# liruiw/GA-DDPG

Measured on AMD Instinct MI355X. Metric: DDPG grad-steps/sec (B=256, N=1024 pts), higher is better.
Workload: dtype f32 (3xbf16-split products, f32 accumulate)

## Files before the change

ga-ddpg_amd/csrc/gemm.hip:

```cpp
#include "common.hpp"
#include <mutex>
#include <type_traits>
#include <string.h>

typedef float f32x16 __attribute__((ext_vector_type(16)));

#ifndef GAD_STREAM_STORE_AUX
#define GAD_STREAM_STORE_AUX 0
#endif

#define KT 32

__device__ __forceinline__ float4 f4zero() { return make_float4(0.f, 0.f, 0.f, 0.f); }
__device__ __forceinline__ float4 f4sel(bool c, float4 a, float4 b) {
    return make_float4(c ? a.x : b.x, c ? a.y : b.y, c ? a.z : b.z, c ? a.w : b.w);
}
__device__ __forceinline__ float4 ldg4(const float* p) { return *reinterpret_cast<const float4*>(p); }

typedef unsigned gad_u32x4 __attribute__((ext_vector_type(4)));
__device__ __forceinline__ float4 buf_ld4(__amdgpu_buffer_rsrc_t r, int vo, int so) {
    const gad_u32x4 u = __builtin_amdgcn_raw_buffer_load_b128(r, vo, so, 0);
    return make_float4(__uint_as_float(u.x), __uint_as_float(u.y), __uint_as_float(u.z), __uint_as_float(u.w));
}
__device__ __forceinline__ float buf_ld(__amdgpu_buffer_rsrc_t r, int vo, int so) {
// ... 205 lines not shown
        if (d.gmode == 0) {
            g = d.G[(size_t)rr * d.g_pitch + ch];
        } else {
            const int grp = d.row_grp[rr];
            g = d.argmax[(size_t)grp * d.c + ch] == r ? d.dout[(size_t)grp * d.c + ch] : 0.f;
        }
        if (d.relu && !d.premasked) {
            const float y = d.scale ? fmaf(z, d.scale[ch], d.shift[ch]) : z;
            g = y > 0.f ? g : 0.f;
        }
        if (d.P) {
            const float w = d.row_w ? d.row_w[rr] : 1.f;
            g = d.P[ch] * g - w * fmaf(d.S[ch], z, d.Q[ch]);
        }
        v[j] = ok ? g : 0.f;
    }
    return make_float4(v[0], v[1], v[2], v[3]);
}

template <bool VEC>
__device__ __forceinline__ DzRaw dz_raw(const DzSrc& d, int r, bool valid, int off, int n, int nmax, int grp) {
    DzRaw o;
    o.z = f4zero(); o.a = make_int4(0, 0, 0, 0);
    if (!VEC) { o.g = dz_scalar4(d, r, valid, off, n, nmax); return o; }
    const int rr = valid ? r : 0;
    const int ch = off + (n < nmax ? n : 0);
    if (d.z) o.z = ldg4(d.z + (size_t)rr * d.z_pitch + ch);
    if (d.gmode == 0) {
        o.g = ldg4(d.G + (size_t)rr * d.g_pitch + ch);
    } else {
        o.a = *reinterpret_cast<const int4*>(d.argmax + (size_t)grp * d.c + ch);
        o.g = ldg4(d.dout + (size_t)grp * d.c + ch);
    }
    return o;
}

template <bool VEC, int VM = VMAX>
__device__ __forceinline__ float4 dz_finish(const DzSrc& d, const DzRaw& raw, int r, bool valid, int n, int nmax, float w,
                                            const float* vec) {
    if (!VEC) return raw.g;
    const bool inside = n < nmax;
    const int nn = inside ? n : 0;
    float4 g = raw.g;
    const float4 z = raw.z;
    if (d.gmode != 0) {
        g.x = raw.a.x == r ? g.x : 0.f; g.y = raw.a.y == r ? g.y : 0.f;
        g.z = raw.a.z == r ? g.z : 0.f; g.w = raw.a.w == r ? g.w : 0.f;
    }
    if (d.relu && !d.premasked) {
        float4 y = z;
        if (d.scale) {
            const float4 s = *reinterpret_cast<const float4*>(vec + nn), t = *reinterpret_cast<const float4*>(vec + VM + nn);
            y.x = fmaf(z.x, s.x, t.x); y.y = fmaf(z.y, s.y, t.y); y.z = fmaf(z.z, s.z, t.z); y.w = fmaf(z.w, s.w, t.w);
        }
        g.x = y.x > 0.f ? g.x : 0.f; g.y = y.y > 0.f ? g.y : 0.f;
        g.z = y.z > 0.f ? g.z : 0.f; g.w = y.w > 0.f ? g.w : 0.f;
    }
    if (d.coef) {
        const float4 P = *reinterpret_cast<const float4*>(vec + 2 * VM + nn);
        const float4 Q = *reinterpret_cast<const float4*>(vec + 3 * VM + nn);
        const float4 S = *reinterpret_cast<const float4*>(vec + 4 * VM + nn);
        g.x = P.x * g.x - w * fmaf(S.x, z.x, Q.x); g.y = P.y * g.y - w * fmaf(S.y, z.y, Q.y);
        g.z = P.z * g.z - w * fmaf(S.z, z.z, Q.z); g.w = P.w * g.w - w * fmaf(S.w, z.w, Q.w);
    }
    return f4sel(valid && inside, g, f4zero());
}

template <int VM = VMAX>
__device__ __forceinline__ void stage_dz_vecs(float* vec, const DzSrc& d, int off, int n) {
    if (!d.premasked) {
        stage_vec(vec, d.scale, off, n, 1.f);
        stage_vec(vec + VM, d.shift, off, n, 0.f);
    }
    for (int i = threadIdx.x; i < n; i += 256) {
        float P, Q, S;
        dz_coef(d, off + i, P, Q, S, first_workgroup());
        vec[2 * VM + i] = P; vec[3 * VM + i] = Q; vec[4 * VM + i] = S;
    }
}

static bool dz_vectorizable(const gad_dz_src& d, const int32_t* off, const int32_t* n_out, int ng) {
    bool ok = (d.z == nullptr || d.z_pitch % 4 == 0) && (d.gmode != 0 || d.g_pitch % 4 == 0) && (d.gmode == 0 || d.c % 4 == 0);
    for (int i = 0; i < ng; ++i) ok = ok && off[i] % 4 == 0 && n_out[i] % 4 == 0 && n_out[i] <= VMAX;
    return ok;
}

template <int DIM> struct PitchT { static constexpr int v = DIM + 1; };
template <int DIM> struct PitchD { static constexpr int v = DIM + 4; };

template <int DIM> __device__ __forceinline__ void unit_T(int u, int& i, int& kk) { i = u >> 3; kk = (u & 7) << 2; }
template <int DIM> __device__ __forceinline__ void unit_D(int u, int& kk, int& i) { kk = u / (DIM / 4); i = (u % (DIM / 4)) << 2; }

template <int DIM> __device__ __forceinline__ void store_T(float* t, int i, int kk, float4 v) {
    constexpr int P = PitchT<DIM>::v;
    t[(kk + 0) * P + i] = v.x; t[(kk + 1) * P + i] = v.y; t[(kk + 2) * P + i] = v.z; t[(kk + 3) * P + i] = v.w;
}
template <int DIM> __device__ __forceinline__ void store_D(float* t, int kk, int i, float4 v) {
    constexpr int P = PitchD<DIM>::v;
    *reinterpret_cast<float4*>(t + kk * P + i) = v;
}

template <int TM, int TN, int PA, int PB>
__device__ __forceinline__ void mfma_ktile(const float* __restrict__ As, const float* __restrict__ Bs, int am0,
                                           int bn0, int lane, f32x16 (&acc)[TM][TN]) {
    const int l31 = lane & 31, half = lane >> 5;
    constexpr int CH = 4, NCH = KT / 2 / CH;
    const float* ap = As + half * PA + am0 + l31;
    const float* bp = Bs + half * PB + bn0 + l31;
    float a[2][CH][TM], b[2][CH][TN];
    auto fetch = [&](int c, int buf) {
#pragma unroll
        for (int s = 0; s < CH; ++s) {
#pragma unroll
            for (int tm = 0; tm < TM; ++tm) a[buf][s][tm] = ap[(2 * (c * CH + s)) * PA + tm * 32];
#pragma unroll
            for (int tn = 0; tn < TN; ++tn) b[buf][s][tn] = bp[(2 * (c * CH + s)) * PB + tn * 32];
        }
    };
    fetch(0, 0);
#pragma unroll
    for (int c = 0; c < NCH; ++c) {
        if (c + 1 < NCH) fetch(c + 1, (c + 1) & 1);
        __builtin_amdgcn_sched_barrier(0);
#pragma unroll
        for (int s = 0; s < CH; ++s)
#pragma unroll
            for (int tm = 0; tm < TM; ++tm)
#pragma unroll
                for (int tn = 0; tn < TN; ++tn)
                    acc[tm][tn] = __builtin_amdgcn_mfma_f32_32x32x2f32(a[c & 1][s][tm], b[c & 1][s][tn], acc[tm][tn], 0, 0, 0);
    }
}

__device__ __forceinline__ int acc_row(int v, int half) { return (v & 3) + 8 * (v >> 2) + 4 * half; }

struct PoolEpi {
    unsigned long long* key;
    const int32_t* row_grp;
    const float* gamma;
    int C;
};

__device__ __forceinline__ unsigned pool_ord(float f) {
    const unsigned u = __float_as_uint(f);
    return u ^ ((unsigned)((int)u >> 31) | 0x80000000u);
}

__device__ __forceinline__ void pool_put(unsigned long long* keycol, int g, int C, float v, int row, bool partial) {
    const unsigned long long k = ((unsigned long long)pool_ord(v) << 32) | (unsigned long long)(0xffffffffu - (unsigned)row);
    if (partial) atomicMax(keycol + (size_t)g * C, k);
    else keycol[(size_t)g * C] = k;
}

struct PoolRun { int g; int part; float v; int row; };

template <int NC>
__device__ __forceinline__ void pool_rows(const float* zt, int pitch, int cstride, int i, int e, int row_base, const float (&sgn)[NC],
                                          float (&best)[NC], int (&brow)[NC]) {
    int r = i;
    for (; r + 2 <= e; r += 2) {
        float z0[NC], z1[NC];
#pragma unroll
        for (int c = 0; c < NC; ++c) { z0[c] = zt[r * pitch + c * cstride] * sgn[c]; z1[c] = zt[(r + 1) * pitch + c * cstride] * sgn[c]; }
#pragma unroll
        for (int c = 0; c < NC; ++c) {
            bool t = z0[c] > best[c]; best[c] = t ? z0[c] : best[c]; brow[c] = t ? row_base + r : brow[c];
            t = z1[c] > best[c]; best[c] = t ? z1[c] : best[c]; brow[c] = t ? row_base + r + 1 : brow[c];
        }
    }
    if (r < e) {
#pragma unroll
        for (int c = 0; c < NC; ++c) {
            const float z0 = zt[r * pitch + c * cstride] * sgn[c];
            const bool t = z0 > best[c]; best[c] = t ? z0 : best[c]; brow[c] = t ? row_base + r : brow[c];
        }
    }
}

__device__ __forceinline__ void pool_scan32(const float* zt, int pitch, int gl, int row_base, float sgn, PoolRun& c,
                                            unsigned long long* keycol, int C) {
    const int lane = threadIdx.x & 63;
    const int prev = __shfl_up(gl, 1, 64);
    const bool st = lane == 0 ? gl != c.g : gl != prev;
    const unsigned m = (unsigned)__ballot(st);
    int i = 0;
    while (i < 32) {
        if ((m >> i) & 1u) {
            if (c.g >= 0) pool_put(keycol, c.g, C, c.v, c.row, c.part != 0);
            c.g = __builtin_amdgcn_readlane(gl, i); c.part = 0; c.v = -INFINITY; c.row = row_base + i;
        }
        const unsigned rest = i < 31 ? m >> (i + 1) : 0u;
        const int e = rest ? i + 1 + __builtin_ctz(rest) : 32;
        if (c.g >= 0) {
            const float sg1[1] = {sgn};
            float bv[1] = {c.v};
            int br[1] = {c.row};
            pool_rows<1>(zt, pitch, 0, i, e, row_base, sg1, bv, br);
            c.v = bv[0]; c.row = br[0];
        }
        i = e;
    }
}

template <int NC>
__device__ __forceinline__ void pool_tile64(const float* zt, int pitch, int cstride, int gl, int row0, int n_live,
                                            const float (&sgn)[NC], int wave, int nw, int g_before, int g_after,
                                            unsigned long long* keycol, int C) {
    const int lane = threadIdx.x & 63;
    const int prev = __shfl_up(gl, 1, 64);
    const bool st = (lane == 0 || gl != prev) && lane < n_live;
    unsigned long long m = __ballot(st);
    int k = 0;
    while (m) {
        const int i = __builtin_ctzll(m);
        m &= m - 1;
        const int e = m ? __builtin_ctzll(m) : n_live;
        if ((k++ % nw) != wave) continue;
        const int g = __builtin_amdgcn_readlane(gl, i);
        float best[NC];
        int brow[NC];
#pragma unroll
        for (int c = 0; c < NC; ++c) { best[c] = -INFINITY; brow[c] = row0 + i; }
        pool_rows<NC>(zt, pitch, cstride, i, e, row0, sgn, best, brow);
        const bool partial = (i == 0 && g == g_before) || (e == n_live && g == g_after);
#pragma unroll
        for (int c = 0; c < NC; ++c) pool_put(keycol + c * cstride, g, C, best[c], brow[c], partial);
    }
}

struct Groups {
    int n; int aoff[GAD_MAX_GROUPS]; int woff[GAD_MAX_GROUPS]; int ooff[GAD_MAX_GROUPS]; int nout[GAD_MAX_GROUPS];
};

template <int WM, int WN, int TN, bool STORE = false>
__device__ __forceinline__ void block_column_atomics(float* red, const float (&c0)[TN], const float (&c1)[TN], int lane,
                                                     int wm, int wn, int col0, int col_limit, double* out0,
                                                     double* out1) {
    constexpr int BN = WN * TN * 32;
    __syncthreads();
#pragma unroll
    for (int tn = 0; tn < TN; ++tn) {
        const float s0 = c0[tn] + __shfl_xor(c0[tn], 32, 64);
        const float s1 = c1[tn] + __shfl_xor(c1[tn], 32, 64);
        if (lane < 32) {
            const int cl = wn * TN * 32 + tn * 32 + lane;
            red[wm * BN + cl] = s0;
            red[(WM + wm) * BN + cl] = s1;
        }
    }
    __syncthreads();
    const int tid = threadIdx.x;
    if (tid < BN && col0 + tid < col_limit) {
        float s0 = 0.f, s1 = 0.f;
#pragma unroll
        for (int w = 0; w < WM; ++w) { s0 += red[w * BN + tid]; s1 += red[(WM + w) * BN + tid]; }
        if (STORE) {
            out0[col0 + tid] = (double)s0;
            out1[col0 + tid] = (double)s1;
        } else {
            atomic_add_f64(out0 + col0 + tid, (double)s0);
            atomic_add_f64(out1 + col0 + tid, (double)s1);
        }
    }
}

template <int WM, int WN, int TM, int TN, int XM, bool POOL, bool DET = false>
__global__ __launch_bounds__(256) void gemm_fwd_kernel(XSrc x, Groups gr, const int32_t* __restrict__ n_rows_dev,
                                                        int n_rows_static, const float* __restrict__ row_w,
                                                        const float* __restrict__ W, int Kp,
                                                        float* __restrict__ zout, int zout_pitch,
                                                        double* __restrict__ stat_sum,
                                                        double* __restrict__ stat_sq, int stat_stride, PoolEpi pe,
                                                        unsigned long long* __restrict__ ts) {
    KTimer kt(ts);
    constexpr int BM = WM * TM * 32, BN = WN * TN * 32;
    constexpr int PA = PitchT<BM>::v, PB = PitchT<BN>::v;
    constexpr int UA = BM * 8 / 256, UB = BN * 8 / 256;
    constexpr int TILE = KT * PA + KT * PB;
    constexpr int SM = ((TILE + 3) & ~3) + 2 * BM + 2 * VMAX;
    static_assert(TILE >= 2 * WM * BN, "reduction scratch must fit in the tile LDS");
    __shared__ __attribute__((aligned(16))) float smem[SM];
    float* As = smem;
    float* Bs = smem + KT * PA;
    float* wS = smem + ((TILE + 3) & ~3);
    int32_t* ptS = reinterpret_cast<int32_t*>(wS + BM);
    float* sv = wS + 2 * BM;
    float* tv = sv + VMAX;

    const int tid = threadIdx.x, lane = tid & 63, wave = tid >> 6;
    const int wm = wave / WN, wn = wave % WN;
    const int g = blockIdx.z;
    const int zoff = gr.aoff[g], n_out = gr.nout[g], ooff = gr.ooff[g];
    const float* Wg = W + gr.woff[g];
    const int n0 = blockIdx.y * BN;
    if (n0 >= n_out) return;
    const int n_rows = n_rows_dev ? min(*n_rows_dev, n_rows_static) : n_rows_static;
    if ((int)(blockIdx.x * BM) >= n_rows) return;
    const int nk = (Kp + KT - 1) / KT;
    const int bulk = XM == 0 ? x.c_in : x.feat_c;

    float csum[TN], csq[TN];
#pragma unroll
    for (int t = 0; t < TN; ++t) { csum[t] = 0.f; csq[t] = 0.f; }

    int row0 = blockIdx.x * BM;
    XRaw ra[UA];
    float4 rb[UB];
    auto load_tile = [&](int kt) {
        const int k0 = kt * KT;
        const bool tail = k0 + KT > bulk;
#pragma unroll
        for (int it = 0; it < UA; ++it) {
            int i, kk; unit_T<BM>(it * 256 + tid, i, kk);
            const int r = row0 + i;
            const bool ok = r < n_rows && (k0 + kk < Kp);
            ra[it] = x_raw<XM>(x, r, ok, zoff, k0 + kk, tail, XM == 1 ? ptS[i] : 0);
        }
#pragma unroll
        for (int it = 0; it < UB; ++it) {
            int j, kk; unit_T<BN>(it * 256 + tid, j, kk);
            const int n = n0 + j;
            const bool ok = n < n_out && (k0 + kk < Kp);
            rb[it] = ldg4(Wg + (size_t)(ok ? n : 0) * Kp + (ok ? k0 + kk : 0));
        }
    };
    auto store_tile = [&](int kt) {
        const int k0 = kt * KT;
#pragma unroll
        for (int it = 0; it < UA; ++it) {
            int i, kk; unit_T<BM>(it * 256 + tid, i, kk);
            const int r = row0 + i;
            const bool ok = r < n_rows && (k0 + kk < Kp);
            store_T<BM>(As, i, kk, x_finish<XM>(x, ra[it], ok, k0 + kk, sv, tv));
        }
#pragma unroll
        for (int it = 0; it < UB; ++it) {
            int j, kk; unit_T<BN>(it * 256 + tid, j, kk);
            const bool ok = (n0 + j) < n_out && (k0 + kk < Kp);
            store_T<BN>(Bs, j, kk, f4sel(ok, rb[it], f4zero()));
        }
    };
    bool preloaded = false;
    if (XM == 0) { load_tile(0); preloaded = true; }
    if (XM == 0 && x.affine) stage_affine<256>(sv, tv, x, zoff, x.c_in);
    for (; row0 < n_rows; row0 += gridDim.x * BM) {
        f32x16 acc[TM][TN];
#pragma unroll
        for (int a = 0; a < TM; ++a)
#pragma unroll
            for (int b = 0; b < TN; ++b)
#pragma unroll
// ... 296 lines not shown
                    an = *reinterpret_cast<const float4*>(As + 8 * (j + 1));
                    bn0 = *reinterpret_cast<const float4*>(Bs + 8 * (j + 1));
                    bn1 = *reinterpret_cast<const float4*>(Bs + 32 * P + 8 * (j + 1));
                }
                acc[0] = __builtin_amdgcn_mfma_f32_32x32x2f32(a4.x, b0.x, acc[0], 0, 0, 0);
                acc[1] = __builtin_amdgcn_mfma_f32_32x32x2f32(a4.x, b1.x, acc[1], 0, 0, 0);
                acc[0] = __builtin_amdgcn_mfma_f32_32x32x2f32(a4.y, b0.y, acc[0], 0, 0, 0);
                acc[1] = __builtin_amdgcn_mfma_f32_32x32x2f32(a4.y, b1.y, acc[1], 0, 0, 0);
                acc[0] = __builtin_amdgcn_mfma_f32_32x32x2f32(a4.z, b0.z, acc[0], 0, 0, 0);
                acc[1] = __builtin_amdgcn_mfma_f32_32x32x2f32(a4.z, b1.z, acc[1], 0, 0, 0);
                acc[0] = __builtin_amdgcn_mfma_f32_32x32x2f32(a4.w, b0.w, acc[0], 0, 0, 0);
                acc[1] = __builtin_amdgcn_mfma_f32_32x32x2f32(a4.w, b1.w, acc[1], 0, 0, 0);
                a4 = an; b0 = bn0; b1 = bn1;
            }
            if (kt + 1 < nk) write_lds(kt + 1, nxtc);
            if (kt + 3 < nk) load_regs(kt + 3, nxtc);
            __syncthreads();
        };
        for (int kt = 0; kt < nk; kt += 2) {
            ktile(kt, S1);
            if (kt + 1 < nk) ktile(kt + 1, S0);
        }
        GAD_WPH(3);
        if (SP) {
#pragma unroll
            for (int t = 0; t < 2; ++t)
#pragma unroll
                for (int v = 0; v < 16; ++v) acc[t][v] = (v & 1) ? an[t][v] - acc[t][v] : acc[t][v] - an[t][v];
        }
        if (XM == 1) {
#pragma unroll
            for (int t = 0; t < 2; ++t) {
                const float* wx = W + (size_t)(n0 + wn * 64 + t * 32 + l31) * Kp + x.feat_c;
                const float w0 = wx[0], w1 = wx[1], w2 = wx[2];
#pragma unroll
                for (int v = 0; v < 16; ++v) {
                    const float4 q = *reinterpret_cast<const float4*>(dxS + 4 * (wm * 32 + acc_row(v, half)));
                    acc[t][v] = fmaf(q.x, w0, fmaf(q.y, w1, fmaf(q.z, w2, acc[t][v])));
                }
            }
        }
        if (POOL) {
            float* zt = smem;
#pragma unroll
            for (int t = 0; t < 2; ++t)
#pragma unroll
                for (int v = 0; v < 16; ++v) zt[(wm * 32 + acc_row(v, half)) * 129 + wn * 64 + t * 32 + l31] = acc[t][v];
            __syncthreads();
            const int gb = __builtin_amdgcn_readfirstlane(pg_before), ga = __builtin_amdgcn_readfirstlane(pg_after);
            pool_tile64<2>(zt + lane, 129, 64, pgl, row0, min(64, n_rows - row0), psgn, wave, 4, gb, ga, pe.key + n0 + lane, pe.C);
        }
        if (SP) {
#pragma unroll
        for (int t = 0; t < 2; ++t) {
            const int n = n0 + wn * 64 + t * 32 + l31;
            const int vzo = (4 * half * zout_pitch + n) * 4;
#pragma unroll
            for (int v = 0; v < 16; ++v)
                __builtin_amdgcn_raw_buffer_store_b32(__float_as_uint(acc[t][v]), zo_, vzo, (row0 + wm * 32 + (v & 3) + 8 * (v >> 2)) * zo_pitch4, 0);
        }
        __builtin_amdgcn_sched_barrier(0);
#pragma unroll
        for (int t = 0; t < 2; ++t) {
            float s1 = 0.f, s2 = 0.f;
#pragma unroll
            for (int v = 0; v < 16; ++v) {
                const float w = wS[wm * 32 + acc_row(v, half)];
                const float zv = acc[t][v];
                s1 = fmaf(w, zv, s1);
                s2 = fmaf(w * zv, zv, s2);
            }
            csum[t] += s1;
            csq[t] += s2;
        }
        } else {
#pragma unroll
        for (int t = 0; t < 2; ++t) {
            const int n = n0 + wn * 64 + t * 32 + l31;
            const int vzo = (4 * half * zout_pitch + n) * 4;
            float s1 = 0.f, s2 = 0.f;
#pragma unroll
            for (int v = 0; v < 16; ++v) {
                const int il = wm * 32 + acc_row(v, half);
                const float zv = acc[t][v];
                __builtin_amdgcn_raw_buffer_store_b32(__float_as_uint(zv), zo_, vzo, (row0 + wm * 32 + (v & 3) + 8 * (v >> 2)) * zo_pitch4, 0);
                const float w = wS[il];
                s1 = fmaf(w, zv, s1);
                s2 = fmaf(w * zv, zv, s2);
            }
            csum[t] += s1;
            csq[t] += s2;
        }
        }
        GAD_WPH(4);
    }
    if (stat_sum) {
        const int rep = blockIdx.x % GAD_STAT_REPLICAS;
        block_column_atomics<2, 2, 2>(smem, csum, csq, lane, wm, wn, n0, n_out, stat_sum + (size_t)rep * stat_stride,
                                      stat_sq + (size_t)rep * stat_stride);
    }
#ifdef GAD_W_PHASES
    __asm__ volatile("s_waitcnt vmcnt(0)" ::: "memory");
    GAD_WPH(5);
    GAD_WPH_STORE(ts);
    GAD_WKL_STORE(ts);
#endif
}

static int g_opt_fwd_wide = 1;
static int g_opt_dx_wide = 1, g_opt_dw_wide = 1;
static int g_opt_bwd_fused = 1;
static int g_opt_fwd_bn_prologue = 1;
static int g_opt_bwd_wide = 0;
static int g_opt_bwd_wide_slab = 4;
static int g_opt_dw_wide_wgs = 256;
static bool fits_i32_bytes(long long rows, int pitch_a, int pitch_b, int pitch_c, int pitch_d);
static bool fwd_wideable(const gad_gemm_fwd_args& a) {
    if (g_opt_deterministic || !g_opt_fwd_wide || a.n_groups != 1 || a.zin_off[0] != 0 || a.w_off[0] != 0 || a.out_off[0] != 0) return false;
    if (!fits_i32_bytes(a.n_rows, a.mode == 1 ? a.feat_c : a.zin_pitch, a.zout ? a.zout_pitch : 0, 0, 0)) return false;
    if (a.n_rows < 2048 || a.n_out[0] % 128 != 0 || a.ones_col >= 0) return false;
    if (a.mode == 2) return false;
    if (a.mode == 1)
        return g_opt_fwd_wide != 2 && !a.pool_key && a.act_c == 0 && a.feat_c % 32 == 0 && a.feat_c >= 32 && a.feat_c <= 512 &&
               a.Kp == ((a.feat_c + 3 + 7) & ~7);
    if (a.Kp % 32 != 0 || a.Kp > 512 || a.Kp != a.c_in) return false;
    return !a.extra && a.scale && a.shift && a.relu;
}
static bool fits_i32_bytes(long long rows, int pitch_a, int pitch_b, int pitch_c, int pitch_d) {
    int p = pitch_a > pitch_b ? pitch_a : pitch_b;
    p = p > pitch_c ? p : pitch_c;
    p = p > pitch_d ? p : pitch_d;
    return rows * (long long)p * 4 <= (1ll << 31);
}

template <int KJ, int TN, int XM, bool POOL, bool SP = false>
__global__ __launch_bounds__(512, 2) void gemm_fwd_stream_kernel(XSrc x, const int32_t* __restrict__ n_rows_dev,
                                                                  int n_rows_static, const float* __restrict__ row_w,
                                                                  const float* __restrict__ W, float* __restrict__ zout,
                                                                  double* __restrict__ stat_sum,
                                                                  double* __restrict__ stat_sq, int stat_stride, PoolEpi pe,
                                                                  unsigned long long* __restrict__ ts) {
#ifdef GAD_X_PHASES
    const long long kt_start = __builtin_readcyclecounter();
#else
    KTimer kt(ts);
#endif
    constexpr int KP = 8 * KJ, NO = 32 * TN, PW = KP + 4;
    constexpr bool RE = XM >= 2;
    constexpr int PK = RE ? XM - 1 : 0;
    constexpr bool ACT = XM == 0 || RE, GATHER = XM == 1 || RE;
    constexpr int NG = RE ? PK : KJ;
    static_assert(!RE || (KJ == 8 && !POOL), "recomputed input: 64 channels");
    static_assert(!SP || (XM == 0 && KJ == 8), "split-bf16: ACT input, 64 channels");
    constexpr int PB = 2 * KP + 16;
    __shared__ __attribute__((aligned(16))) float Ws[SP ? 3 * NO * PB / 4 : NO * PW];
    __shared__ __attribute__((aligned(16))) float sv[KP], tv[KP];
    __shared__ float red[2 * 8 * NO];
    __shared__ float pz[POOL ? 8 * 32 * 64 : 1];
    static_assert(!POOL || TN == 4, "pooled epilogue: 128 output columns");
    const int tid = threadIdx.x, lane = tid & 63;
    const int wave = __builtin_amdgcn_readfirstlane(tid >> 6);
    const int l31 = lane & 31, half = lane >> 5;
    const int n_rows = n_rows_dev ? min(*n_rows_dev, n_rows_static) : n_rows_static;
    const int n_slabs = (n_rows + 31) >> 5;
#if GAD_X_PHASES == 2
    long long st1, st2, st3, st4;
    __asm__ volatile("s_waitcnt lgkmcnt(0)" ::: "memory");
    GAD_PH_STAMP(st1);
#endif
    int stride = gridDim.x * 8;
    int slab = wave * gridDim.x + blockIdx.x;
    int slab_end = n_slabs;
    if (POOL) {
        const int nw = gridDim.x * 8, base = n_slabs / nw, rem = n_slabs - base * nw;
        slab_end = slab * base + min(slab, rem) + base + (slab < rem ? 1 : 0);
        slab = slab * base + min(slab, rem);
        stride = 1;
    }
    const bool store_z = zout != nullptr;
    const __amdgpu_buffer_rsrc_t zrsrc =
        __builtin_amdgcn_make_buffer_rsrc(store_z ? zout : const_cast<float*>(W), 0, store_z ? gad_nbytes(n_rows, NO * 4) : 0, 0x00020000);
    const int zlane = (4 * half * NO + l31) * 4;
    float psgn[2];
    PoolRun prun[2];
    const int range0 = slab * 32;
    int g_after = -1;
    if (POOL && slab < slab_end) {
        const int g0 = pe.row_grp[range0];
        const int part0 = range0 > 0 && pe.row_grp[range0 - 1] == g0;
        if (slab_end * 32 < n_rows) g_after = pe.row_grp[slab_end * 32];
#pragma unroll
        for (int p = 0; p < 2; ++p) {
            psgn[p] = pe.gamma[p * 64 + lane] < 0.f ? -1.f : 1.f;
            prun[p].g = g0; prun[p].part = part0; prun[p].v = -INFINITY; prun[p].row = range0;
        }
    }

    f32x2 csum[TN], csq[TN];
#pragma unroll
    for (int t = 0; t < TN; ++t) { csum[t] = f32x2{0.f, 0.f}; csq[t] = f32x2{0.f, 0.f}; }

    XRaw ra[NG], rn[NG];
    float4 w1f[RE ? 2 : 1][RE ? PK : 1];
    if (RE) {
#pragma unroll
        for (int b = 0; b < 2; ++b)
#pragma unroll
            for (int j = 0; j < PK; ++j) w1f[b][j] = ldg4(x.pre_W + (size_t)(32 * b + l31) * x.pre_Kp + 8 * j + 4 * half);
    }
    int pt_nxt = 0;
    auto load_pt = [&](int sl) {
        const int r = min(sl * 32 + l31, max(n_rows - 1, 0));
        return (GATHER && sl < n_slabs) ? x.row_pt[r] : 0;
    };
    auto load_slab = [&](int sl, int pt, XRaw (&dst)[NG]) {
        const int r = min(sl < n_slabs ? sl * 32 + l31 : 0, max(n_rows - 1, 0));
        if (GATHER) {
            struct F3 { float x, y, z; } __attribute__((packed, aligned(4)));
            const float4 f = ldg4(x.feat + (size_t)pt * 4);
            const F3 p = *reinterpret_cast<const F3*>(x.src_xyz + (size_t)pt * 3);
            const int grp = x.row_grp[r];
            float q0 = p.x, q1 = p.y, q2 = p.z;
            if (x.ctr_xyz) {
                const F3 c = *reinterpret_cast<const F3*>(x.ctr_xyz + (size_t)grp * 3);
                q0 = __fsub_rn(q0, c.x); q1 = __fsub_rn(q1, c.y); q2 = __fsub_rn(q2, c.z);
            }
            float a0 = 0.f, a1 = 0.f, a2 = 0.f, a3 = 0.f, a4 = 0.f, a5 = 0.f;
            if (x.action) {
                const float* ap = x.action + (size_t)(grp / x.gps) * 6;
                const F3 u = *reinterpret_cast<const F3*>(ap), v = *reinterpret_cast<const F3*>(ap + 3);
                a0 = u.x; a1 = u.y; a2 = u.z; a3 = v.x; a4 = v.y; a5 = v.z;
            }
#pragma unroll
            for (int j = 0; j < NG; ++j) {
                dst[j].a = f;
                if (j == 0) dst[j].s = make_float4(q0, q1, q2, a0);
                else dst[j].s = half ? make_float4(a5, 0.f, 0.f, 0.f) : make_float4(a1, a2, a3, a4);
            }
            return;
        }
#pragma unroll
        for (int j = 0; j < NG; ++j)
            dst[j] = x_raw<GATHER ? 1 : 0>(x, r, true, 0, SP ? 16 * (j >> 1) + 8 * half + 4 * (j & 1) : 8 * j + 4 * half, GATHER, pt);
    };
    auto lds_b = [&](int j, float4 (&b4)[TN]) {
#pragma unroll
        for (int t = 0; t < TN; ++t) b4[t] = *reinterpret_cast<const float4*>(Ws + (t * 32 + l31) * PW + 8 * j + 4 * half);
    };
    {
        const int pt0 = load_pt(slab);
        load_slab(slab, pt0, ra);
        pt_nxt = load_pt(slab + stride);
    }
    {
        constexpr int UNITS = NO * KJ * 2, UW = (UNITS + 511) / 512;
        float4 wr[UW];
#pragma unroll
        for (int it = 0; it < UW; ++it) {
            const int u = it * 512 + tid;
            wr[it] = ldg4(W + (size_t)(u < UNITS ? u : 0) * 4);
        }
#if GAD_X_PHASES == 2
        GAD_PH_STAMP(st2);
        __asm__ volatile("s_waitcnt vmcnt(0)" ::: "memory");
        GAD_PH_STAMP(st3);
#endif
        if (ACT && tid < KP) {
            float sc, sh;
            if (x.bn.stat_sum) gad_bn_fin_channel(x.bn, tid, blockIdx.x == 0, sc, sh);
            else { sc = x.scale[tid]; sh = x.shift[tid]; }
            sv[tid] = sc; tv[tid] = sh;
        }
#pragma unroll
        for (int it = 0; it < UW; ++it) {
            const int u = it * 512 + tid;
            const int n = u / (KJ * 2), c = (u % (KJ * 2)) * 4;
            if (SP) {
                unsigned h0, m0, l0, h1, m1, l1;
                gad_split2(wr[it].x, wr[it].y, h0, m0, l0);
                gad_split2(wr[it].z, wr[it].w, h1, m1, l1);
                unsigned char* wp = reinterpret_cast<unsigned char*>(Ws) + n * PB + c * 2;
                if (u < UNITS) {
                    *reinterpret_cast<uint2*>(wp) = make_uint2(h0, h1);
                    *reinterpret_cast<uint2*>(wp + NO * PB) = make_uint2(m0, m1);
                    *reinterpret_cast<uint2*>(wp + 2 * NO * PB) = make_uint2(l0, l1);
                }
            } else if (u < UNITS) *reinterpret_cast<float4*>(Ws + n * PW + c) = wr[it];
        }
    }
    __syncthreads();
#if GAD_X_PHASES == 2
    GAD_PH_STAMP(st4);
    if (ts && lane == 0) {
        auto c16 = [&](long long t) { const long long d = (t - kt_start) >> 2; return (unsigned long long)(d > 65535 ? 65535 : d); };
        ts[2 * (blockIdx.x * 8 + wave)] = c16(st1) | (c16(st2) << 16) | (c16(st3) << 32) | (c16(st4) << 48);
    }
#endif

#ifdef GAD_X_PHASES
    long long tA = 0, tB = 0, tC = 0, ph_top = 0, ph_mfma = 0, ph_epi = 0;
    int ph_n = 0;
    long long tP, tS;
    GAD_PH_STAMP(tP);
    tS = (long long)kt_start;
#endif
    for (; slab < slab_end; slab += stride) {
        load_slab(slab + stride, pt_nxt, rn);
        pt_nxt = load_pt(slab + 2 * stride);
        float4 w4[4];
#pragma unroll
        for (int q = 0; q < 4; ++q) {
            const int r0 = slab * 32 + 8 * q + 4 * half;
            w4[q] = row_w ? ldg4(row_w + (r0 + 3 < n_rows_static ? r0 : 0)) : make_float4(1.f, 1.f, 1.f, 1.f);
        }
        if (slab * 32 + 32 > n_rows) {
#pragma unroll
            for (int q = 0; q < 4; ++q) {
                float* wq = &w4[q].x;
#pragma unroll
                for (int e = 0; e < 4; ++e) wq[e] = (slab * 32 + 8 * q + 4 * half + e < n_rows) ? wq[e] : 0.f;
            }
        }
        int gl = -1;
        if (POOL) { const int rr = slab * 32 + l31; gl = rr < n_rows ? pe.row_grp[rr] : -1; }
        __asm__ volatile("" ::: "memory");
        f32x16 acc[TN];
#pragma unroll
        for (int t = 0; t < TN; ++t)
#pragma unroll
            for (int v = 0; v < 16; ++v) acc[t][v] = 0.f;
        float4 bn[TN];
        if (!SP) lds_b(0, bn);
        GAD_PH_STAMP(tA);
        if (SP) {
            const unsigned char* wp = reinterpret_cast<const unsigned char*>(Ws) + l31 * PB + 16 * half;
            constexpr int NS = SP ? KJ / 2 : 1;
            gad_u32x4 AH[NS], AM[NS], AL[NS];
#pragma unroll
            for (int sg = 0; sg < NS; ++sg) {
                unsigned ah[4], am[4], al[4];
#pragma unroll
                for (int e = 0; e < 2; ++e) {
                    const int c = 16 * sg + 8 * half + 4 * e;
                    const float4 s4 = *reinterpret_cast<const float4*>(sv + c), t4 = *reinterpret_cast<const float4*>(tv + c);
                    const float4 zr = ra[SP ? 2 * sg + e : 0].a;
                    const float a0 = __builtin_fmaxf(fmaf(zr.x, s4.x, t4.x), 0.f), a1 = __builtin_fmaxf(fmaf(zr.y, s4.y, t4.y), 0.f);
                    const float a2 = __builtin_fmaxf(fmaf(zr.z, s4.z, t4.z), 0.f), a3 = __builtin_fmaxf(fmaf(zr.w, s4.w, t4.w), 0.f);
                    gad_split2(a0, a1, ah[2 * e], am[2 * e], al[2 * e]);
                    gad_split2(a2, a3, ah[2 * e + 1], am[2 * e + 1], al[2 * e + 1]);
                }
                const unsigned sgn = ((sg ^ l31) & 1) ? 0x80008000u : 0u;
                AH[sg] = gad_u32x4{ah[0] ^ sgn, ah[1] ^ sgn, ah[2] ^ sgn, ah[3] ^ sgn};
                AM[sg] = gad_u32x4{am[0] ^ sgn, am[1] ^ sgn, am[2] ^ sgn, am[3] ^ sgn};
                AL[sg] = gad_u32x4{al[0] ^ sgn, al[1] ^ sgn, al[2] ^ sgn, al[3] ^ sgn};
            }
#pragma unroll
            for (int pp = 0; pp < TN / 2; ++pp) {
                f32x16 an[2];
#pragma unroll
                for (int i = 0; i < 2; ++i)
#pragma unroll
                    for (int v = 0; v < 16; ++v) an[i][v] = 0.f;
#pragma unroll
                for (int sg = 0; sg < NS; ++sg) {
                    gad_u32x4 BH[2], BM[2], BL[2];
#pragma unroll
                    for (int i = 0; i < 2; ++i) {
                        const unsigned char* q = wp + (2 * pp + i) * 32 * PB + 32 * sg;
                        BH[i] = *reinterpret_cast<const gad_u32x4*>(q);
                        BM[i] = *reinterpret_cast<const gad_u32x4*>(q + NO * PB);
                        BL[i] = *reinterpret_cast<const gad_u32x4*>(q + 2 * NO * PB);
                    }
#define GAD_SPLIT_MFMA(A, B)                                                                                                   \
                    _Pragma("unroll") for (int i = 0; i < 2; ++i) {                                                             \
                        if (sg & 1) an[i] = __builtin_amdgcn_mfma_f32_32x32x16_bf16(gad_as_bf16x8(A[sg]), gad_as_bf16x8(B[i]), an[i], 0, 0, 0); \
                        else acc[2 * pp + i] = __builtin_amdgcn_mfma_f32_32x32x16_bf16(gad_as_bf16x8(A[sg]), gad_as_bf16x8(B[i]), acc[2 * pp + i], 0, 0, 0); \
                    }
                    GAD_SPLIT_MFMA(AL, BH) GAD_SPLIT_MFMA(AH, BL) GAD_SPLIT_MFMA(AM, BM)
                    GAD_SPLIT_MFMA(AM, BH) GAD_SPLIT_MFMA(AH, BM) GAD_SPLIT_MFMA(AH, BH)
#undef GAD_SPLIT_MFMA
                }
#pragma unroll
                for (int i = 0; i < 2; ++i)
#pragma unroll
                    for (int v = 0; v < 16; ++v) acc[2 * pp + i][v] = (v & 1) ? an[i][v] - acc[2 * pp + i][v] : acc[2 * pp + i][v] - an[i][v];
            }
        }
        f32x16 zacc[RE ? 2 : 1];
        if (RE) {
#pragma unroll
            for (int b = 0; b < 2; ++b)
#pragma unroll
                for (int v = 0; v < 16; ++v) zacc[b][v] = 0.f;
#pragma unroll
            for (int j = 0; j < PK; ++j) {
                const float4 xb = x_finish<1>(x, ra[j], true, 8 * j + 4 * half, sv, tv);
#pragma unroll
                for (int b = 0; b < 2; ++b) zacc[b] = __builtin_amdgcn_mfma_f32_32x32x2f32(w1f[b][j].x, xb.x, zacc[b], 0, 0, 0);
#pragma unroll
                for (int b = 0; b < 2; ++b) zacc[b] = __builtin_amdgcn_mfma_f32_32x32x2f32(w1f[b][j].y, xb.y, zacc[b], 0, 0, 0);
#pragma unroll
                for (int b = 0; b < 2; ++b) zacc[b] = __builtin_amdgcn_mfma_f32_32x32x2f32(w1f[b][j].z, xb.z, zacc[b], 0, 0, 0);
#pragma unroll
                for (int b = 0; b < 2; ++b) zacc[b] = __builtin_amdgcn_mfma_f32_32x32x2f32(w1f[b][j].w, xb.w, zacc[b], 0, 0, 0);
            }
        }
#pragma unroll
        for (int j = 0; j < (SP ? 0 : KJ); ++j) {
            float4 b4[TN];
#pragma unroll
            for (int t = 0; t < TN; ++t) b4[t] = bn[t];
            float4 a4;
            if (ACT) {
                const float4 s4 = *reinterpret_cast<const float4*>(sv + 8 * j + 4 * half);
                const float4 t4 = *reinterpret_cast<const float4*>(tv + 8 * j + 4 * half);
                float4 zr;
                if (RE) zr = make_float4(zacc[j >> 2][4 * (j & 3)], zacc[j >> 2][4 * (j & 3) + 1], zacc[j >> 2][4 * (j & 3) + 2],
                                         zacc[j >> 2][4 * (j & 3) + 3]);
                else zr = ra[RE ? 0 : j].a;
                const f32x2 lo = f32x2{zr.x, zr.y} * f32x2{s4.x, s4.y} + f32x2{t4.x, t4.y};
                const f32x2 hi = f32x2{zr.z, zr.w} * f32x2{s4.z, s4.w} + f32x2{t4.z, t4.w};
                a4 = make_float4(__builtin_fmaxf(lo.x, 0.f), __builtin_fmaxf(lo.y, 0.f), __builtin_fmaxf(hi.x, 0.f),
                                 __builtin_fmaxf(hi.y, 0.f));
            } else {
                a4 = x_finish<1>(x, ra[RE ? 0 : j], true, 8 * j + 4 * half, sv, tv);
            }
            if (j + 1 < KJ) lds_b(j + 1, bn);
#pragma unroll
            for (int t = 0; t < TN; ++t) acc[t] = __builtin_amdgcn_mfma_f32_32x32x2f32(a4.x, b4[t].x, acc[t], 0, 0, 0);
#pragma unroll
            for (int t = 0; t < TN; ++t) acc[t] = __builtin_amdgcn_mfma_f32_32x32x2f32(a4.y, b4[t].y, acc[t], 0, 0, 0);
#pragma unroll
            for (int t = 0; t < TN; ++t) acc[t] = __builtin_amdgcn_mfma_f32_32x32x2f32(a4.z, b4[t].z, acc[t], 0, 0, 0);
#pragma unroll
            for (int t = 0; t < TN; ++t) acc[t] = __builtin_amdgcn_mfma_f32_32x32x2f32(a4.w, b4[t].w, acc[t], 0, 0, 0);
        }
        GAD_PH_STAMP(tB);
        const int zrow = slab * 32 * NO * 4;
        if (POOL) {
            float* zt = pz + wave * (32 * 64);
#pragma unroll
            for (int p = 0; p < 2; ++p) {
#pragma unroll
                for (int v = 0; v < 16; ++v) {
                    zt[acc_row(v, half) * 64 + l31] = acc[2 * p][v];
                    zt[acc_row(v, half) * 64 + 32 + l31] = acc[2 * p + 1][v];
                }
                pool_scan32(zt + lane, 64, gl, slab * 32, psgn[p], prun[p], pe.key + p * 64 + lane, pe.C);
            }
        }
#pragma unroll
        for (int v = 0; v < 16; v += 2) {
            const int rb = ((v & 3) + 8 * (v >> 2)) * NO * 4;
            const f32x2 wr = f32x2{(&w4[v >> 2].x)[v & 3], (&w4[v >> 2].x)[(v & 3) + 1]};
#pragma unroll
            for (int t = 0; t < TN; ++t) {
                const f32x2 zv = f32x2{acc[t][v], acc[t][v + 1]};
                if (store_z) {
                    __builtin_amdgcn_raw_buffer_store_b32(__float_as_uint(acc[t][v]), zrsrc, zlane + t * 128, zrow + rb, GAD_STREAM_STORE_AUX);
                    __builtin_amdgcn_raw_buffer_store_b32(__float_as_uint(acc[t][v + 1]), zrsrc, zlane + t * 128, zrow + rb + NO * 4, GAD_STREAM_STORE_AUX);
                }
                const f32x2 wz = wr * zv;
                csum[t] += wz;
                csq[t] += wz * zv;
            }
        }
#pragma unroll
        for (int j = 0; j < NG; ++j) ra[j] = rn[j];
#ifdef GAD_X_PHASES
        GAD_PH_STAMP(tC);
        ph_top += tA - tP; ph_mfma += tB - tA; ph_epi += tC - tB; tP = tC; ++ph_n;
#endif
    }
#ifdef GAD_X_PHASES
    if (ts && lane == 0) {
        const unsigned w = blockIdx.x * 8 + wave;
        if (GAD_X_PHASES != 2) ts[2 * w] = ((unsigned long long)ph_mfma << 32) | (unsigned long long)(ph_epi & 0xffffffffu);
        ts[2 * w + 1] = ((unsigned long long)ph_top << 32) | ((unsigned long long)(tP - tS) & 0xffffff00u) | (unsigned long long)ph_n;
    }
#endif
    if (POOL && range0 < slab_end * 32) {
#pragma unroll
        for (int p = 0; p < 2; ++p)
            if (prun[p].g >= 0)
                pool_put(pe.key + p * 64 + lane, prun[p].g, pe.C, prun[p].v, prun[p].row, prun[p].part != 0 || prun[p].g == g_after);
    }
    if (stat_sum) {
#pragma unroll
        for (int t = 0; t < TN; ++t) {
            const float c0 = csum[t].x + csum[t].y, c1 = csq[t].x + csq[t].y;
            const float s0 = c0 + __shfl_xor(c0, 32, 64);
            const float s1 = c1 + __shfl_xor(c1, 32, 64);
            if (lane < 32) { red[wave * NO + t * 32 + lane] = s0; red[(8 + wave) * NO + t * 32 + lane] = s1; }
        }
        __syncthreads();
        if (tid < NO) {
            float s0 = 0.f, s1 = 0.f;
#pragma unroll
            for (int w = 0; w < 8; ++w) { s0 += red[w * NO + tid]; s1 += red[(8 + w) * NO + tid]; }
            const int rep = blockIdx.x % GAD_STAT_REPLICAS;
            atomic_add_f64(stat_sum + (size_t)rep * stat_stride + tid, (double)s0);
            atomic_add_f64(stat_sq + (size_t)rep * stat_stride + tid, (double)s1);
        }
    }
}

#define SK_NW 8
#define SK_CH 6
#define SK_SP 36
#define SK_KCAP (8 * SK_NW * SK_CH * SK_MAXCH)
#define SK_MAXCH 3
template <int NW>
__global__ __launch_bounds__(64 * NW) void gemm_fwd_skinny_kernel(XSrc x, Groups gr, int n_rows,
                                                                     const float* __restrict__ row_w,
                                                                     const float* __restrict__ W, int Kp,
                                                                     float* __restrict__ zout, int zout_pitch,
                                                                     double* __restrict__ stat_sum,
                                                                     double* __restrict__ stat_sq, int stat_stride, unsigned long long* __restrict__ ts) {
    KTimer kt(ts);
    __shared__ __attribute__((aligned(16))) float stA[NW * 32 * SK_SP], stW[NW * 32 * SK_SP];
    __shared__ __attribute__((aligned(16))) float sv[SK_KCAP], tv[SK_KCAP];
    float* const part = stA;
    static_assert(32 * SK_SP >= 16 * 64, "partial tile must fit the wavefront's stage");
    const int tid = threadIdx.x, lane = tid & 63;
    const int wave = __builtin_amdgcn_readfirstlane(tid >> 6);
    const int l31 = lane & 31, half = lane >> 5;
    const int g = blockIdx.z;
    const int zoff = gr.aoff[g], n_out = gr.nout[g], ooff = gr.ooff[g];
    const int n0 = blockIdx.x * 32, row0 = blockIdx.y * 32;
    if (n0 >= n_out) return;
    const float* Wg = W + gr.woff[g] + (size_t)min(n0 + l31, n_out - 1) * Kp + 4 * half;
    const int r = min(row0 + l31, max(n_rows - 1, 0));
    const int nj = Kp >> 3;
    const int per = (nj + NW - 1) / NW;
    const int j0 = wave * per, j1 = min(nj, j0 + per);

    f32x16 acc;
#pragma unroll
    for (int v = 0; v < 16; ++v) acc[v] = 0.f;
    float* const myA = stA + wave * (32 * SK_SP);
    float* const myW = stW + wave * (32 * SK_SP);
    const int rsub = lane >> 3, chunk = lane & 7;
    const float* pa[4];
    const float* pw[4];
#pragma unroll
    for (int i = 0; i < 4; ++i) {
        pa[i] = x.zin + (size_t)min(row0 + rsub + 8 * i, max(n_rows - 1, 0)) * x.zin_pitch + zoff + 4 * chunk;
        pw[i] = W + gr.woff[g] + (size_t)min(n0 + rsub + 8 * i, n_out - 1) * Kp + 4 * chunk;
    }
    auto staged = [&](int jb) { return jb + 4 <= j1 && 8 * (jb + 4) <= x.c_in; };
    float4 ga[4], gw[4];
    auto load_blk = [&](int jb) {
#pragma unroll
        for (int i = 0; i < 4; ++i) { ga[i] = ldg4(pa[i] + 8 * jb); gw[i] = ldg4(pw[i] + 8 * jb); }
    };
    if (j0 < j1 && staged(j0)) load_blk(j0);
    if (x.bn.stat_sum) {
        const bool writer = blockIdx.x == 0 && blockIdx.y == 0;
        for (int i = tid; i < x.c_in; i += 64 * NW) {
            float sc, sh;
            gad_bn_fin_channel(x.bn, i, writer, sc, sh);
            sv[i] = sc;
            tv[i] = sh;
        }
    } else if (x.affine) stage_affine<64 * NW>(sv, tv, x, zoff, x.c_in);
    __syncthreads();
    for (int jb = j0; jb < j1; jb += 4) {
        if (staged(jb)) {
#pragma unroll
            for (int i = 0; i < 4; ++i) {
                *reinterpret_cast<float4*>(myA + (rsub + 8 * i) * SK_SP + 4 * chunk) = ga[i];
                *reinterpret_cast<float4*>(myW + (rsub + 8 * i) * SK_SP + 4 * chunk) = gw[i];
            }
            if (jb + 4 < j1 && staged(jb + 4)) load_blk(jb + 4);
            __builtin_amdgcn_fence(__ATOMIC_RELEASE, "wavefront");
            __builtin_amdgcn_wave_barrier();
            __builtin_amdgcn_fence(__ATOMIC_ACQUIRE, "wavefront");
#pragma unroll
            for (int u = 0; u < 4; ++u) {
                XRaw raw;
                raw.a = *reinterpret_cast<const float4*>(myA + l31 * SK_SP + 8 * u + 4 * half);
                raw.s = f4zero();
                const float4 a4 = x_finish<0>(x, raw, true, 8 * (jb + u) + 4 * half, sv, tv);
                const float4 b4 = *reinterpret_cast<const float4*>(myW + l31 * SK_SP + 8 * u + 4 * half);
                acc = __builtin_amdgcn_mfma_f32_32x32x2f32(a4.x, b4.x, acc, 0, 0, 0);
                acc = __builtin_amdgcn_mfma_f32_32x32x2f32(a4.y, b4.y, acc, 0, 0, 0);
                acc = __builtin_amdgcn_mfma_f32_32x32x2f32(a4.z, b4.z, acc, 0, 0, 0);
                acc = __builtin_amdgcn_mfma_f32_32x32x2f32(a4.w, b4.w, acc, 0, 0, 0);
            }
            __builtin_amdgcn_fence(__ATOMIC_RELEASE, "wavefront");
            __builtin_amdgcn_wave_barrier();
        } else {
            const int je = min(jb + 4, j1);
            XRaw ra[4];
            float4 rb[4];
#pragma unroll
            for (int u = 0; u < 4; ++u) {
                const int j = min(jb + u, nj - 1);
                const int col = 8 * j + 4 * half;
                ra[u] = x_raw<0>(x, r, true, zoff, col, col + 4 > x.c_in, 0);
                rb[u] = ldg4(Wg + 8 * j);
            }
            if (jb + 4 < j1 && staged(jb + 4)) load_blk(jb + 4);
#pragma unroll
            for (int u = 0; u < 4; ++u) {
                if (jb + u < je) {
                    const float4 a4 = x_finish<0>(x, ra[u], true, 8 * (jb + u) + 4 * half, sv, tv);
                    const float4 b4 = rb[u];
                    acc = __builtin_amdgcn_mfma_f32_32x32x2f32(a4.x, b4.x, acc, 0, 0, 0);
                    acc = __builtin_amdgcn_mfma_f32_32x32x2f32(a4.y, b4.y, acc, 0, 0, 0);
                    acc = __builtin_amdgcn_mfma_f32_32x32x2f32(a4.z, b4.z, acc, 0, 0, 0);
                    acc = __builtin_amdgcn_mfma_f32_32x32x2f32(a4.w, b4.w, acc, 0, 0, 0);
                }
            }
        }
    }
#pragma unroll
    for (int v = 0; v < 16; ++v) part[wave * (32 * SK_SP) + v * 64 + lane] = acc[v];
    __syncthreads();
    if (wave != 0) return;
#pragma unroll
    for (int w = 1; w < NW; ++w)
#pragma unroll
        for (int v = 0; v < 16; ++v) acc[v] += part[w * (32 * SK_SP) + v * 64 + lane];
    const int n = n0 + l31;
    float s1 = 0.f, s2 = 0.f;
#pragma unroll
    for (int v = 0; v < 16; ++v) {
        const int rr = row0 + acc_row(v, half);
        const float zv = acc[v];
        const bool live = rr < n_rows;
        if (live && n < n_out) zout[(size_t)rr * zout_pitch + ooff + n] = zv;
        const float w = live ? (row_w ? row_w[rr] : 1.f) : 0.f;
        s1 = fmaf(w, zv, s1);
        s2 = fmaf(w * zv, zv, s2);
    }
    if (stat_sum) {
        s1 += __shfl_xor(s1, 32, 64);
// ... 3322 lines not shown
```

Before: 395.2.

## Pool max directly from MFMA accumulator registers instead of LDS transpose

Replaces the pooled epilogue, which staged accumulator tiles through a per-wave LDS buffer and scanned rows per lane. The new path does the segmented argmax straight on the MFMA accumulator registers, using masked octets and a permlane32 swap to merge the two half-waves. It applies the gamma sign with an XOR on the sign bit and drops the large shared pz array, which cuts LDS traffic and may improve occupancy. It also specializes the ACT-input load path to read float4 directly, and makes the slab bounds wave-uniform. The register-resident version adds more VGPR pressure and complicates tie-breaking between rows.

```diff
diff --git a/ga-ddpg_amd/csrc/gemm.hip b/ga-ddpg_amd/csrc/gemm.hip
--- a/ga-ddpg_amd/csrc/gemm.hip
+++ b/ga-ddpg_amd/csrc/gemm.hip
@@ -381,8 +381,6 @@
     else keycol[(size_t)g * C] = k;
 }
 
-struct PoolRun { int g; int part; float v; int row; };
-
 template <int NC>
 __device__ __forceinline__ void pool_rows(const float* zt, int pitch, int cstride, int i, int e, int row_base, const float (&sgn)[NC],
                                           float (&best)[NC], int (&brow)[NC]) {
@@ -406,8 +404,45 @@
     }
 }
 
-__device__ __forceinline__ void pool_scan32(const float* zt, int pitch, int gl, int row_base, float sgn, PoolRun& c,
-                                            unsigned long long* keycol, int C) {
+struct PoolRegs { int g; int part; float v[4]; int row[4]; };
+
+template <bool MASKED>
+__device__ __forceinline__ void pool_regs_octet(const f32x16 (&zs)[4], int v0, unsigned oct, int row8, PoolRegs& c) {
+#pragma unroll
+    for (int j = 0; j < 4; ++j) {
+        bool in = true;
+        if (MASKED)
+            in = __builtin_amdgcn_inverse_ballot_w64((((oct >> j) & 1u) ? 0xffffffffull : 0ull) |
+                                                     (((oct >> (4 + j)) & 1u) ? 0xffffffff00000000ull : 0ull));
+#pragma unroll
+        for (int t = 0; t < 4; ++t) {
+            const float z = zs[t][v0 + j];
+            const bool tk = z > c.v[t] && in;
+            c.v[t] = tk ? z : c.v[t]; c.row[t] = tk ? row8 + j : c.row[t];
+        }
+    }
+}
+
+__device__ __forceinline__ void pool_regs_close(const PoolRegs& c, int half, unsigned long long* keycol, int C, bool partial) {
+    float bv[4];
+    int br[4];
+#pragma unroll
+    for (int t = 0; t < 4; ++t) {
+        const int row = c.row[t] + 4 * half;
+        const unsigned vb = __float_as_uint(c.v[t]);
+        const float ov = __uint_as_float(__builtin_amdgcn_permlane32_swap(vb, vb, false, false)[1]);
+        const int orow = (int)__builtin_amdgcn_permlane32_swap((unsigned)row, (unsigned)row, false, false)[1];
+        const bool tk = ov > c.v[t] || (ov == c.v[t] && orow < row);
+        bv[t] = tk ? ov : c.v[t]; br[t] = tk ? orow : row;
+    }
+    if (half == 0) {
+#pragma unroll
+        for (int t = 0; t < 4; ++t) pool_put(keycol + 32 * t, c.g, C, bv[t], br[t], partial);
+    }
+}
+
+__device__ __forceinline__ void pool_slab_regs(const f32x16 (&zs)[4], int gl, int row_base, int half, PoolRegs& c,
+                                               unsigned long long* keycol, int C) {
     const int lane = threadIdx.x & 63;
     const int prev = __shfl_up(gl, 1, 64);
     const bool st = lane == 0 ? gl != c.g : gl != prev;
@@ -415,17 +450,21 @@
     int i = 0;
     while (i < 32) {
         if ((m >> i) & 1u) {
-            if (c.g >= 0) pool_put(keycol, c.g, C, c.v, c.row, c.part != 0);
-            c.g = __builtin_amdgcn_readlane(gl, i); c.part = 0; c.v = -INFINITY; c.row = row_base + i;
+            if (c.g >= 0) pool_regs_close(c, half, keycol, C, c.part != 0);
+            c.g = __builtin_amdgcn_readlane(gl, i); c.part = 0;
+#pragma unroll
+            for (int t = 0; t < 4; ++t) { c.v[t] = -INFINITY; c.row[t] = row_base + i - 4 * half; }
         }
         const unsigned rest = i < 31 ? m >> (i + 1) : 0u;
         const int e = rest ? i + 1 + __builtin_ctz(rest) : 32;
         if (c.g >= 0) {
-            const float sg1[1] = {sgn};
-            float bv[1] = {c.v};
-            int br[1] = {c.row};
-            pool_rows<1>(zt, pitch, 0, i, e, row_base, sg1, bv, br);
-            c.v = bv[0]; c.row = br[0];
+            const unsigned seg = (e < 32 ? (1u << e) - 1u : 0xffffffffu) & ~((1u << i) - 1u);
+#pragma unroll
+            for (int q = 0; q < 4; ++q) {
+                const unsigned oct = (seg >> (8 * q)) & 0xffu;
+                if (oct == 0xffu) pool_regs_octet<false>(zs, 4 * q, oct, row_base + 8 * q, c);
+                else if (oct) pool_regs_octet<true>(zs, 4 * q, oct, row_base + 8 * q, c);
+            }
         }
         i = e;
     }
@@ -1028,11 +1067,11 @@
     constexpr int NG = RE ? PK : KJ;
     static_assert(!RE || (KJ == 8 && !POOL), "recomputed input: 64 channels");
     static_assert(!SP || (XM == 0 && KJ == 8), "split-bf16: ACT input, 64 channels");
+    static_assert(XM != 0 || KJ == 8, "ACT input read from memory: 64 channels");
     constexpr int PB = 2 * KP + 16;
     __shared__ __attribute__((aligned(16))) float Ws[SP ? 3 * NO * PB / 4 : NO * PW];
     __shared__ __attribute__((aligned(16))) float sv[KP], tv[KP];
     __shared__ float red[2 * 8 * NO];
-    __shared__ float pz[POOL ? 8 * 32 * 64 : 1];
     static_assert(!POOL || TN == 4, "pooled epilogue: 128 output columns");
     const int tid = threadIdx.x, lane = tid & 63;
     const int wave = __builtin_amdgcn_readfirstlane(tid >> 6);
@@ -1049,26 +1088,26 @@
     int slab_end = n_slabs;
     if (POOL) {
         const int nw = gridDim.x * 8, base = n_slabs / nw, rem = n_slabs - base * nw;
-        slab_end = slab * base + min(slab, rem) + base + (slab < rem ? 1 : 0);
-        slab = slab * base + min(slab, rem);
+        slab_end = __builtin_amdgcn_readfirstlane(slab * base + min(slab, rem) + base + (slab < rem ? 1 : 0));
+        slab = __builtin_amdgcn_readfirstlane(slab * base + min(slab, rem));
         stride = 1;
     }
     const bool store_z = zout != nullptr;
     const __amdgpu_buffer_rsrc_t zrsrc =
         __builtin_amdgcn_make_buffer_rsrc(store_z ? zout : const_cast<float*>(W), 0, store_z ? gad_nbytes(n_rows, NO * 4) : 0, 0x00020000);
     const int zlane = (4 * half * NO + l31) * 4;
-    float psgn[2];
-    PoolRun prun[2];
+    unsigned psgn[4];
+    PoolRegs prun;
     const int range0 = slab * 32;
     int g_after = -1;
     if (POOL && slab < slab_end) {
         const int g0 = pe.row_grp[range0];
-        const int part0 = range0 > 0 && pe.row_grp[range0 - 1] == g0;
         if (slab_end * 32 < n_rows) g_after = pe.row_grp[slab_end * 32];
-#pragma unroll
-        for (int p = 0; p < 2; ++p) {
-            psgn[p] = pe.gamma[p * 64 + lane] < 0.f ? -1.f : 1.f;
-            prun[p].g = g0; prun[p].part = part0; prun[p].v = -INFINITY; prun[p].row = range0;
+        prun.g = g0; prun.part = range0 > 0 && pe.row_grp[range0 - 1] == g0;
+#pragma unroll
+        for (int t = 0; t < 4; ++t) {
+            psgn[t] = pe.gamma[t * 32 + l31] < 0.f ? 0x80000000u : 0u;
+            prun.v[t] = -INFINITY; prun.row[t] = range0 - 4 * half;
         }
     }
 
@@ -1115,9 +1154,15 @@
             }
             return;
         }
+        if (XM == 0) {
+            const float* zr = x.zin + (size_t)r * x.zin_pitch + (SP ? 8 : 4) * half;
+#pragma unroll
+            for (int j = 0; j < NG; ++j) dst[j].a = ldg4(zr + (SP ? 16 * (j >> 1) + 4 * (j & 1) : 8 * j));
+            return;
+        }
 #pragma unroll
         for (int j = 0; j < NG; ++j)
-            dst[j] = x_raw<GATHER ? 1 : 0>(x, r, true, 0, SP ? 16 * (j >> 1) + 8 * half + 4 * (j & 1) : 8 * j + 4 * half, GATHER, pt);
+            dst[j] = x_raw<GATHER ? 1 : 0>(x, r, true, 0, 8 * j + 4 * half, GATHER, pt);
     };
     auto lds_b = [&](int j, float4 (&b4)[TN]) {
 #pragma unroll
@@ -1313,33 +1358,34 @@
         }
         GAD_PH_STAMP(tB);
         const int zrow = slab * 32 * NO * 4;
-        if (POOL) {
-            float* zt = pz + wave * (32 * 64);
-#pragma unroll
-            for (int p = 0; p < 2; ++p) {
-#pragma unroll
-                for (int v = 0; v < 16; ++v) {
-                    zt[acc_row(v, half) * 64 + l31] = acc[2 * p][v];
-                    zt[acc_row(v, half) * 64 + 32 + l31] = acc[2 * p + 1][v];
-                }
-                pool_scan32(zt + lane, 64, gl, slab * 32, psgn[p], prun[p], pe.key + p * 64 + lane, pe.C);
-            }
-        }
-#pragma unroll
-        for (int v = 0; v < 16; v += 2) {
-            const int rb = ((v & 3) + 8 * (v >> 2)) * NO * 4;
-            const f32x2 wr = f32x2{(&w4[v >> 2].x)[v & 3], (&w4[v >> 2].x)[(v & 3) + 1]};
-#pragma unroll
-            for (int t = 0; t < TN; ++t) {
-                const f32x2 zv = f32x2{acc[t][v], acc[t][v + 1]};
-                if (store_z) {
+        if (store_z) {
+#pragma unroll
+            for (int v = 0; v < 16; v += 2) {
+                const int rb = ((v & 3) + 8 * (v >> 2)) * NO * 4;
+#pragma unroll
+                for (int t = 0; t < TN; ++t) {
                     __builtin_amdgcn_raw_buffer_store_b32(__float_as_uint(acc[t][v]), zrsrc, zlane + t * 128, zrow + rb, GAD_STREAM_STORE_AUX);
                     __builtin_amdgcn_raw_buffer_store_b32(__float_as_uint(acc[t][v + 1]), zrsrc, zlane + t * 128, zrow + rb + NO * 4, GAD_STREAM_STORE_AUX);
                 }
+            }
+        }
+#pragma unroll
+        for (int v = 0; v < 16; v += 2) {
+            const f32x2 wr = f32x2{(&w4[v >> 2].x)[v & 3], (&w4[v >> 2].x)[(v & 3) + 1]};
+#pragma unroll
+            for (int t = 0; t < TN; ++t) {
+                const f32x2 zv = f32x2{acc[t][v], acc[t][v + 1]};
                 const f32x2 wz = wr * zv;
                 csum[t] += wz;
                 csq[t] += wz * zv;
             }
+        }
+        if constexpr (POOL) {
+#pragma unroll
+            for (int t = 0; t < TN; ++t)
+#pragma unroll
+                for (int v = 0; v < 16; ++v) acc[t][v] = __uint_as_float(__float_as_uint(acc[t][v]) ^ psgn[t]);
+            pool_slab_regs(acc, gl, slab * 32, half, prun, pe.key + l31, pe.C);
         }
 #pragma unroll
         for (int j = 0; j < NG; ++j) ra[j] = rn[j];
@@ -1356,10 +1402,7 @@
     }
 #endif
     if (POOL && range0 < slab_end * 32) {
-#pragma unroll
-        for (int p = 0; p < 2; ++p)
-            if (prun[p].g >= 0)
-                pool_put(pe.key + p * 64 + lane, prun[p].g, pe.C, prun[p].v, prun[p].row, prun[p].part != 0 || prun[p].g == g_after);
+        if (prun.g >= 0) pool_regs_close(prun, half, pe.key + l31, pe.C, prun.part != 0 || prun.g == g_after);
     }
     if (stat_sum) {
 #pragma unroll
```

After: 393.0. Within noise of the previous version (-0.6%).
